# diffqc/dqc

Measured on AMD Instinct MI355X. Metric: SCF iterations/sec (Fock build + XC grid) per GPU, cc-pVDZ 20-atom, higher is better.
Workload: dtype f64

## Files before the change

dqc_amd/csrc/jk.hip:

```cpp
#include <cstdlib>

#include "common.hpp"

namespace dqc {

DQC_DEV void decode_tri(long long t, int &a, int &b) {
    long long r = (long long)((sqrt(8.0 * (double)t + 1.0) - 1.0) * 0.5);
    while (r * (r + 1) / 2 > t) r--;
    while ((r + 1) * (r + 2) / 2 <= t) r++;
    a = (int)r;
    b = (int)(t - r * (r + 1) / 2);
}

DQC_DEV void tile_load_patch(const double *__restrict__ tiles, int IJ, int KL, int I, int J, int K, int L, int r0, int c0, double2 &a0, double2 &b0, double2 &a1, double2 &b1, double2 &a2,
                             double2 &b2, double2 &a3, double2 &b3, const TileLay &ly) {
    const bool dr = I == J, dc = K == L;
    const double *tp = tiles + tile_base(I, J, K, KL, ly);
    const bool trunc = I == ly.last && ly.wl < 8;
    if (!dr && !dc) {
        if (trunc && r0 >= 8 * ly.wl) {
            a0 = b0 = a1 = b1 = a2 = b2 = a3 = b3 = make_double2(0.0, 0.0);
            return;
        }
        const double *q = tp + r0 * 64 + c0;
// ... 116 lines not shown
    if ((long long)blockIdx.x < ntiles) JKM_LOAD(blockIdx.x)
    for (long long T = blockIdx.x; T < ntiles; T += gridDim.x) {
        int IJ, KL, I, J, K, L;
        decode_tri(T, IJ, KL);
        decode_tri(IJ, I, J);
        decode_tri(KL, K, L);
        const double f = (I == J ? 0.5 : 1.0) * (K == L ? 0.5 : 1.0) * (IJ == KL ? 0.5 : 1.0);
        const int kk = c0 >> 3, l0 = c0 & 7, ii = r0 >> 3, j0 = r0 & 7;
        double g[4][4];
        g[0][0] = na0.x; g[0][1] = na0.y; g[0][2] = nb0.x; g[0][3] = nb0.y;
        g[1][0] = na1.x; g[1][1] = na1.y; g[1][2] = nb1.x; g[1][3] = nb1.y;
        g[2][0] = na2.x; g[2][1] = na2.y; g[2][2] = nb2.x; g[2][3] = nb2.y;
        g[3][0] = na3.x; g[3][1] = na3.y; g[3][2] = nb3.x; g[3][3] = nb3.y;
        if (T + gridDim.x < ntiles) JKM_LOAD(T + gridDim.x)
        if (NK) {
#pragma unroll
            for (int r = 0; r < 4; r++) {
                *reinterpret_cast<double2 *>(&s_g[(r0 + r) * LDT + c0]) = make_double2(g[r][0], g[r][1]);
                *reinterpret_cast<double2 *>(&s_g[(r0 + r) * LDT + c0 + 2]) = make_double2(g[r][2], g[r][3]);
            }
            const int blk = t >> 6, e = t & 63, x = e >> 3, y = e & 7;
            const int R = (blk & 1) ? I : J, Cb = (blk & 2) ? L : K;
#pragma unroll
            for (int q = 0; q < NK; q++) s_d[blk][x * 9 + y][q] = Dk[q * n2 + (size_t)(R * 8 + x) * npad + Cb * 8 + y];
        }
        for (int q = 0; q < nj; q++) {
            const double *dklp = Dj + q * n2 + (size_t)(K * 8 + kk) * npad + L * 8 + l0;
            const double *dijp = Dj + q * n2 + (size_t)(I * 8 + ii) * npad + J * 8 + j0;
            double dkl[4], dij[4];
#pragma unroll
            for (int c = 0; c < 4; c++) { dkl[c] = dklp[c]; dij[c] = dijp[c]; }
            double rs[4] = {0, 0, 0, 0}, cs[4] = {0, 0, 0, 0};
#pragma unroll
            for (int r = 0; r < 4; r++)
#pragma unroll
                for (int c = 0; c < 4; c++) {
                    rs[r] += g[r][c] * dkl[c];
                    cs[c] += g[r][c] * dij[r];
                }
#pragma unroll
            for (int r = 0; r < 4; r++) {
                double v = rs[r];
                v += __shfl_xor(v, 1); v += __shfl_xor(v, 2); v += __shfl_xor(v, 4); v += __shfl_xor(v, 8);
                rs[r] = v;
            }
#pragma unroll
            for (int c = 0; c < 4; c++) {
                double v = cs[c];
                v += __shfl_xor(v, 16); v += __shfl_xor(v, 32);
                cs[c] = v;
            }
            double *Jq = Jacc + q * n2;
            if ((lane & 15) == 0) {
#pragma unroll
                for (int r = 0; r < 4; r++) acc_add(&Jq[(size_t)(I * 8 + ii) * npad + J * 8 + j0 + r], 2.0 * f * rs[r], dsc);
            }
            if (lane < 16) {
#pragma unroll
                for (int c = 0; c < 4; c++) s_col[q & 1][wave][c0 + c] = cs[c];
            }
            __syncthreads();
            if (t < 64) {
                const double v = s_col[q & 1][0][t] + s_col[q & 1][1][t] + s_col[q & 1][2][t] + s_col[q & 1][3][t];
                acc_add(&Jq[(size_t)(K * 8 + (t >> 3)) * npad + L * 8 + (t & 7)], 2.0 * f * v, dsc);
            }
        }
        if (NK) {
            if (nj == 0) __syncthreads();
            const int o = t >> 2, pg = t & 3, x = o >> 3, y = o & 7, yh = y >> 2;
            double k1[NKD], k2[NKD], k3[NKD], k4[NKD];
#pragma unroll
            for (int q = 0; q < NK; q++) k1[q] = k2[q] = k3[q] = k4[q] = 0.0;
#pragma unroll 1
            for (int u = 0; u < 2; u++) {
                const int qq = pg + 4 * u, q4 = pg + 4 * (u ^ yh);
#pragma unroll 4
                for (int a = 0; a < 8; a++) {
                    const double g1 = s_g[(x * 8 + a) * LDT + qq * 8 + y], g2 = s_g[(a * 8 + x) * LDT + qq * 8 + y];
                    const double g3 = s_g[(x * 8 + a) * LDT + y * 8 + q4], g4 = s_g[(a * 8 + x) * LDT + y * 8 + q4];
                    if constexpr (NK == 2) {
                        const vd2 d1 = *reinterpret_cast<const vd2 *>(&s_d[0][a * 9 + qq][0]);
                        const vd2 d2 = *reinterpret_cast<const vd2 *>(&s_d[1][a * 9 + qq][0]);
                        const vd2 d3 = *reinterpret_cast<const vd2 *>(&s_d[2][a * 9 + q4][0]);
                        const vd2 d4 = *reinterpret_cast<const vd2 *>(&s_d[3][a * 9 + q4][0]);
                        k1[0] += g1 * d1.x; k1[1] += g1 * d1.y;
                        k2[0] += g2 * d2.x; k2[1] += g2 * d2.y;
                        k3[0] += g3 * d3.x; k3[1] += g3 * d3.y;
                        k4[0] += g4 * d4.x; k4[1] += g4 * d4.y;
                    } else {
#pragma unroll
                        for (int q = 0; q < NK; q++) {
                            k1[q] += g1 * s_d[0][a * 9 + qq][q];
                            k2[q] += g2 * s_d[1][a * 9 + qq][q];
                            k3[q] += g3 * s_d[2][a * 9 + q4][q];
                            k4[q] += g4 * s_d[3][a * 9 + q4][q];
                        }
                    }
                }
            }
#pragma unroll
            for (int q = 0; q < NK; q++) {
                double a1 = k1[q], a2 = k2[q], a3 = k3[q], a4 = k4[q];
                a1 += __shfl_xor(a1, 1); a1 += __shfl_xor(a1, 2);
                a2 += __shfl_xor(a2, 1); a2 += __shfl_xor(a2, 2);
                a3 += __shfl_xor(a3, 1); a3 += __shfl_xor(a3, 2);
                a4 += __shfl_xor(a4, 1); a4 += __shfl_xor(a4, 2);
                if (pg == 0) {
                    double *Kq = Kacc + q * n2;
                    acc_add(&Kq[(size_t)(I * 8 + x) * npad + L * 8 + y], f * a1, dsc);
                    acc_add(&Kq[(size_t)(J * 8 + x) * npad + L * 8 + y], f * a2, dsc);
                    acc_add(&Kq[(size_t)(I * 8 + x) * npad + K * 8 + y], f * a3, dsc);
                    acc_add(&Kq[(size_t)(J * 8 + x) * npad + K * 8 + y], f * a4, dsc);
                }
            }
        }
        __syncthreads();
    }
}

#undef JKM_LOAD
__global__ void jk_multi_prep_kernel(double *__restrict__ work, const double *__restrict__ dmj, int nj, const double *__restrict__ dmk,
                                     int nk, int nao, int npad, unsigned kanti) {
    const size_t n2 = (size_t)npad * npad, nn = (size_t)nao * nao;
    const int nd = nj + nk;
    for (size_t e = (size_t)blockIdx.x * blockDim.x + threadIdx.x; e < n2 * nd; e += (size_t)gridDim.x * blockDim.x) {
        const int q = e / n2;
        const size_t r = e - (size_t)q * n2;
        const int i = r / npad, j = r % npad;
        const double *dm = q < nj ? dmj + (size_t)q * nn : dmk + (size_t)(q - nj) * nn;
        double v = 0.0;
        const bool anti = q >= nj && ((kanti >> (q - nj)) & 1u);
        if (i < nao && j < nao) v = anti ? 0.5 * (dm[(size_t)i * nao + j] - dm[(size_t)j * nao + i]) : 0.5 * (dm[(size_t)i * nao + j] + dm[(size_t)j * nao + i]);
        work[e] = v;
        work[n2 * nd + e] = 0.0;
    }
}

__global__ void jk_multi_finish_kernel(double *__restrict__ J, int nj, double *__restrict__ K, int nk, const double *__restrict__ work,
                                       int nao, int npad, const double *__restrict__ dscp, unsigned kanti) {
    const double dsc = dscp ? *dscp : 0.0;
    const size_t n2 = (size_t)npad * npad, nn = (size_t)nao * nao;
    const double *acc = work + (size_t)(nj + nk) * n2;
    for (size_t e = (size_t)blockIdx.x * blockDim.x + threadIdx.x; e < nn * (nj + nk); e += (size_t)gridDim.x * blockDim.x) {
        const int q = e / nn;
        const size_t r = e - (size_t)q * nn;
        const int i = r / nao, j = r % nao;
        const double a = det_value(acc[q * n2 + (size_t)i * npad + j], dsc), at = det_value(acc[q * n2 + (size_t)j * npad + i], dsc);
        const double v = (q >= nj && ((kanti >> (q - nj)) & 1u)) ? a - at : a + at;
        if (q < nj) J[e] = v;
        else K[e - (size_t)nj * nn] = v;
    }
}

__global__ __launch_bounds__(256, 1) void j_stream_kernel(const double *__restrict__ dscp, const double *__restrict__ tiles,
                                                         double *__restrict__ work, int npad, long long ntiles, long long per_block,
                                                         long long tbeg, int nao) {
    const TileLay ly(nao);
    const double dsc = dscp ? *dscp : 0.0;
    __shared__ double s_col[2][4][64];
    const size_t n2 = (size_t)npad * npad;
    const double *Dp = work;
    double *Jacc = work + n2;
    const int t = threadIdx.x, lane = t & 63, wave = t >> 6;
    const int r0 = 4 * (t >> 4), c0 = 4 * (t & 15);
    const int kk = c0 >> 3, l0 = c0 & 7, ii = r0 >> 3, j0 = r0 & 7;
    const long long T0 = tbeg + (long long)blockIdx.x * per_block, T1 = min(T0 + per_block, ntiles);
    if (T0 >= T1) return;
    int IJ, KL, I, J, K, L;
    decode_tri(T0, IJ, KL);
    decode_tri(IJ, I, J);
    double rsacc[4] = {0, 0, 0, 0}, dij[4];
    {
        const double *dijp = Dp + (size_t)(I * 8 + ii) * npad + J * 8 + j0;
#pragma unroll
        for (int q = 0; q < 4; q++) dij[q] = dijp[q];
    }
    auto flush_rows = [&]() {
        const double fI = (I == J ? 0.5 : 1.0);
#pragma unroll
        for (int r = 0; r < 4; r++) {
            double v = rsacc[r];
            v += __shfl_xor(v, 1); v += __shfl_xor(v, 2); v += __shfl_xor(v, 4); v += __shfl_xor(v, 8);
            if ((lane & 15) == 0) acc_add(&Jacc[(size_t)(I * 8 + ii) * npad + J * 8 + j0 + r], 2.0 * fI * v, dsc);
            rsacc[r] = 0.0;
        }
    };
    int par = 0;
    for (long long T = T0; T < T1; T++, KL++) {
        if (KL > IJ) {
            flush_rows();
            IJ++;
            KL = 0;
            decode_tri(IJ, I, J);
            const double *dijp = Dp + (size_t)(I * 8 + ii) * npad + J * 8 + j0;
#pragma unroll
            for (int q = 0; q < 4; q++) dij[q] = dijp[q];
        }
        decode_tri(KL, K, L);
        const double fk = (K == L ? 0.5 : 1.0) * (IJ == KL ? 0.5 : 1.0);
        const double *dklp = Dp + (size_t)(K * 8 + kk) * npad + L * 8 + l0;
        double dkl[4];
#pragma unroll
        for (int q = 0; q < 4; q++) dkl[q] = fk * dklp[q];
        double cs[4] = {0, 0, 0, 0};
        {
            double2 ta0, tb0, ta1, tb1, ta2, tb2, ta3, tb3;
            tile_load_patch(tiles, IJ, KL, I, J, K, L, r0, c0, ta0, tb0, ta1, tb1, ta2, tb2, ta3, tb3, ly);
#define DQC_JS_ROW(R_, A_, B_)                                                                           \
    rsacc[R_] += A_.x * dkl[0] + A_.y * dkl[1] + B_.x * dkl[2] + B_.y * dkl[3];                          \
    cs[0] += A_.x * dij[R_]; cs[1] += A_.y * dij[R_]; cs[2] += B_.x * dij[R_]; cs[3] += B_.y * dij[R_];
            DQC_JS_ROW(0, ta0, tb0) DQC_JS_ROW(1, ta1, tb1) DQC_JS_ROW(2, ta2, tb2) DQC_JS_ROW(3, ta3, tb3)
#undef DQC_JS_ROW
        }
#pragma unroll
        for (int c = 0; c < 4; c++) {
            double v = cs[c];
            v += __shfl_xor(v, 16); v += __shfl_xor(v, 32);
            cs[c] = v;
        }
        if (lane < 16) {
#pragma unroll
            for (int c = 0; c < 4; c++) s_col[par][wave][c0 + c] = cs[c];
        }
        __syncthreads();
        if (t < 64) {
            const double v = s_col[par][0][t] + s_col[par][1][t] + s_col[par][2][t] + s_col[par][3][t];
            acc_add(&Jacc[(size_t)(K * 8 + (t >> 3)) * npad + L * 8 + (t & 7)], 2.0 * (I == J ? 0.5 : 1.0) * fk * v, dsc);
        }
        par ^= 1;
    }
    flush_rows();
}


__global__ __launch_bounds__(256, 4) void jk_stream_kernel(const double *__restrict__ dscp, const double *__restrict__ tiles,
                                                          double *__restrict__ work, int npad, long long ntiles, long long per_block,
                                                          long long tbeg, int nao) {
    const TileLay ly(nao);
    const double dsc = dscp ? *dscp : 0.0;
    constexpr int LDT = 68;
    __shared__ double s_col[4][64];
    __shared__ __attribute__((aligned(16))) double s_g[64 * LDT];
    __shared__ __attribute__((aligned(16))) double s_d[2][72][2];
    const size_t n2 = (size_t)npad * npad;
    const double *Dp = work;
    double *Jacc = work + n2, *Kacc = work + 2 * n2;
    const int t = threadIdx.x, lane = t & 63, wave = t >> 6;
    const int r0 = 4 * (t >> 4), c0 = 4 * (t & 15);
    const int kk = c0 >> 3, l0 = c0 & 7, ii = r0 >> 3, j0 = r0 & 7;
    const int o = t >> 2, pg = t & 3, x = o >> 3, y = o & 7, yh = y >> 2;
    const long long T0 = tbeg + (long long)blockIdx.x * per_block, T1 = min(T0 + per_block, ntiles);
    if (T0 >= T1) return;
    int IJ, KL, I, J, K, L;
    decode_tri(T0, IJ, KL);
    decode_tri(IJ, I, J);
    decode_tri(KL, K, L);
    double rsacc[4] = {0, 0, 0, 0}, dij[4];
    double k3acc = 0.0, k4acc = 0.0;
    {
        const double *dijp = Dp + (size_t)(I * 8 + ii) * npad + J * 8 + j0;
#pragma unroll
        for (int q = 0; q < 4; q++) dij[q] = dijp[q];
    }
    auto flush_rows = [&]() {
        const double fI = (I == J ? 0.5 : 1.0);
#pragma unroll
        for (int r = 0; r < 4; r++) {
            double v = rsacc[r];
            v += __shfl_xor(v, 1); v += __shfl_xor(v, 2); v += __shfl_xor(v, 4); v += __shfl_xor(v, 8);
            if ((lane & 15) == 0) acc_add(&Jacc[(size_t)(I * 8 + ii) * npad + J * 8 + j0 + r], 2.0 * fI * v, dsc);
            rsacc[r] = 0.0;
        }
    };
    auto flush_k34 = [&]() {
        double a3 = k3acc, a4 = k4acc;
        a3 += __shfl_xor(a3, 1); a3 += __shfl_xor(a3, 2);
        a4 += __shfl_xor(a4, 1); a4 += __shfl_xor(a4, 2);
        if (pg == 0) {
            acc_add(&Kacc[(size_t)(I * 8 + x) * npad + K * 8 + y], a3, dsc);
            acc_add(&Kacc[(size_t)(J * 8 + x) * npad + K * 8 + y], a4, dsc);
        }
        k3acc = k4acc = 0.0;
    };
    for (long long T = T0; T < T1; T++) {
        const double f = (I == J ? 0.5 : 1.0) * (K == L ? 0.5 : 1.0) * (IJ == KL ? 0.5 : 1.0);
        const double fk = (K == L ? 0.5 : 1.0) * (IJ == KL ? 0.5 : 1.0);
        const double *dklp = Dp + (size_t)(K * 8 + kk) * npad + L * 8 + l0;
        double dkl[4];
#pragma unroll
        for (int q = 0; q < 4; q++) dkl[q] = fk * dklp[q];
        double cs[4] = {0, 0, 0, 0};
        {
            double2 ta0, tb0, ta1, tb1, ta2, tb2, ta3, tb3;
            tile_load_patch(tiles, IJ, KL, I, J, K, L, r0, c0, ta0, tb0, ta1, tb1, ta2, tb2, ta3, tb3, ly);
#define DQC_JS_ROW(R_, A_, B_)                                                                           \
    rsacc[R_] += A_.x * dkl[0] + A_.y * dkl[1] + B_.x * dkl[2] + B_.y * dkl[3];                          \
    cs[0] += A_.x * dij[R_]; cs[1] += A_.y * dij[R_]; cs[2] += B_.x * dij[R_]; cs[3] += B_.y * dij[R_]; \
    *reinterpret_cast<double2 *>(&s_g[(r0 + R_) * LDT + c0]) = A_;                                       \
    *reinterpret_cast<double2 *>(&s_g[(r0 + R_) * LDT + c0 + 2]) = B_;
            DQC_JS_ROW(0, ta0, tb0) DQC_JS_ROW(1, ta1, tb1) DQC_JS_ROW(2, ta2, tb2) DQC_JS_ROW(3, ta3, tb3)
#undef DQC_JS_ROW
        }
        {
            const int blk = t >> 6, e = t & 63, xx = e >> 3, yy = e & 7;
            const int R = (blk & 1) ? I : J, Cb = (blk & 2) ? L : K;
            s_d[blk >> 1][xx * 9 + yy][blk & 1] = Dp[(size_t)(R * 8 + xx) * npad + Cb * 8 + yy];
        }
#pragma unroll
        for (int c = 0; c < 4; c++) {
            double v = cs[c];
            v += __shfl_xor(v, 16); v += __shfl_xor(v, 32);
            cs[c] = v;
        }
        if (lane < 16) {
#pragma unroll
            for (int c = 0; c < 4; c++) s_col[wave][c0 + c] = cs[c];
        }
        __syncthreads();
        if (t < 64) {
            const double v = s_col[0][t] + s_col[1][t] + s_col[2][t] + s_col[3][t];
            acc_add(&Jacc[(size_t)(K * 8 + (t >> 3)) * npad + L * 8 + (t & 7)], 2.0 * (I == J ? 0.5 : 1.0) * fk * v, dsc);
        }
        {
            double k1 = 0, k2 = 0, k3 = 0, k4 = 0;
#pragma unroll 1
            for (int u = 0; u < 2; u++) {
                const int q = pg + 4 * u, q4 = pg + 4 * (u ^ yh);
#pragma unroll
                for (int a = 0; a < 8; a++) {
                    typedef double vd2_ __attribute__((ext_vector_type(2)));
                    const vd2_ d12 = *reinterpret_cast<const vd2_ *>(&s_d[0][a * 9 + q][0]);
                    const vd2_ d34 = *reinterpret_cast<const vd2_ *>(&s_d[1][a * 9 + q4][0]);
                    k1 += s_g[(x * 8 + a) * LDT + q * 8 + y] * d12.x;
                    k2 += s_g[(a * 8 + x) * LDT + q * 8 + y] * d12.y;
                    k3 += s_g[(x * 8 + a) * LDT + y * 8 + q4] * d34.x;
                    k4 += s_g[(a * 8 + x) * LDT + y * 8 + q4] * d34.y;
                }
            }
            k1 += __shfl_xor(k1, 1); k1 += __shfl_xor(k1, 2);
            k2 += __shfl_xor(k2, 1); k2 += __shfl_xor(k2, 2);
            if (pg == 0) {
                acc_add(&Kacc[(size_t)(I * 8 + x) * npad + L * 8 + y], f * k1, dsc);
                acc_add(&Kacc[(size_t)(J * 8 + x) * npad + L * 8 + y], f * k2, dsc);
            }
            k3acc += f * k3;
            k4acc += f * k4;
        }
        if (T + 1 < T1) {
            if (KL == IJ) {
                flush_rows();
                flush_k34();
                IJ++;
                KL = 0; K = 0; L = 0;
                decode_tri(IJ, I, J);
                const double *dijp = Dp + (size_t)(I * 8 + ii) * npad + J * 8 + j0;
#pragma unroll
                for (int q = 0; q < 4; q++) dij[q] = dijp[q];
            } else {
                KL++;
                if (L == K) { flush_k34(); K++; L = 0; }
                else L++;
            }
        }
        __syncthreads();
    }
    flush_rows();
    flush_k34();
}

template <int NJ, int NK>
__global__ __launch_bounds__(256, 3) void jk_multi_stream_kernel(const double *__restrict__ dscp, const double *__restrict__ tiles,
                                                                double *__restrict__ work, int npad, long long ntiles,
                                                                long long per_block, int nao) {
    const TileLay ly(nao);
    const double dsc = dscp ? *dscp : 0.0;
    constexpr int LDT = 68;
    __shared__ double s_col[4][64];
    __shared__ __attribute__((aligned(16))) double s_g[64 * LDT];
    __shared__ __attribute__((aligned(16))) double s_d[4][72][NK];
    const size_t n2 = (size_t)npad * npad;
    const double *Dp = work, *Dk = work + (size_t)NJ * n2;
    double *Jacc = work + (size_t)(NJ + NK) * n2, *Kacc = Jacc + (size_t)NJ * n2;
// ... 37 lines not shown
                acc_add(&Kacc[q * n2 + (size_t)(I * 8 + x) * npad + K * 8 + y], a3, dsc);
                acc_add(&Kacc[q * n2 + (size_t)(J * 8 + x) * npad + K * 8 + y], a4, dsc);
            }
            k3acc[q] = k4acc[q] = 0.0;
        }
    };
    for (long long T = T0; T < T1; T++) {
        const double f = (I == J ? 0.5 : 1.0) * (K == L ? 0.5 : 1.0) * (IJ == KL ? 0.5 : 1.0);
        const double fk = (K == L ? 0.5 : 1.0) * (IJ == KL ? 0.5 : 1.0);
        const double *dklp = Dp + (size_t)(K * 8 + kk) * npad + L * 8 + l0;
        double dkl[4];
#pragma unroll
        for (int q = 0; q < 4; q++) dkl[q] = NJ ? fk * dklp[q] : 0.0;
        double cs[4] = {0, 0, 0, 0};
        {
            double2 ta0, tb0, ta1, tb1, ta2, tb2, ta3, tb3;
            tile_load_patch(tiles, IJ, KL, I, J, K, L, r0, c0, ta0, tb0, ta1, tb1, ta2, tb2, ta3, tb3, ly);
#define DQC_JS_ROW(R_, A_, B_)                                                                           \
    if (NJ) {                                                                                            \
        rsacc[R_] += A_.x * dkl[0] + A_.y * dkl[1] + B_.x * dkl[2] + B_.y * dkl[3];                      \
        cs[0] += A_.x * dij[R_]; cs[1] += A_.y * dij[R_]; cs[2] += B_.x * dij[R_]; cs[3] += B_.y * dij[R_]; \
    }                                                                                                    \
    *reinterpret_cast<double2 *>(&s_g[(r0 + R_) * LDT + c0]) = A_;                                       \
    *reinterpret_cast<double2 *>(&s_g[(r0 + R_) * LDT + c0 + 2]) = B_;
            DQC_JS_ROW(0, ta0, tb0) DQC_JS_ROW(1, ta1, tb1) DQC_JS_ROW(2, ta2, tb2) DQC_JS_ROW(3, ta3, tb3)
#undef DQC_JS_ROW
        }
        {
            const int blk = t >> 6, e = t & 63, xx = e >> 3, yy = e & 7;
            const int R = (blk & 1) ? I : J, Cb = (blk & 2) ? L : K;
#pragma unroll
            for (int q = 0; q < NK; q++) s_d[blk][xx * 9 + yy][q] = Dk[q * n2 + (size_t)(R * 8 + xx) * npad + Cb * 8 + yy];
        }
        if (NJ) {
#pragma unroll
            for (int c = 0; c < 4; c++) {
                double v = cs[c];
                v += __shfl_xor(v, 16); v += __shfl_xor(v, 32);
                cs[c] = v;
            }
            if (lane < 16) {
#pragma unroll
                for (int c = 0; c < 4; c++) s_col[wave][c0 + c] = cs[c];
            }
        }
        __syncthreads();
        if (NJ && t < 64) {
            const double v = s_col[0][t] + s_col[1][t] + s_col[2][t] + s_col[3][t];
            acc_add(&Jacc[(size_t)(K * 8 + (t >> 3)) * npad + L * 8 + (t & 7)], 2.0 * (I == J ? 0.5 : 1.0) * fk * v, dsc);
        }
        {
            double k1[NK], k2[NK], k3[NK], k4[NK];
#pragma unroll
            for (int q = 0; q < NK; q++) k1[q] = k2[q] = k3[q] = k4[q] = 0.0;
#pragma unroll 1
            for (int u = 0; u < 2; u++) {
                const int qq = pg + 4 * u, q4 = pg + 4 * (u ^ yh);
#pragma unroll 4
                for (int a = 0; a < 8; a++) {
                    const double g1 = s_g[(x * 8 + a) * LDT + qq * 8 + y], g2 = s_g[(a * 8 + x) * LDT + qq * 8 + y];
                    const double g3 = s_g[(x * 8 + a) * LDT + y * 8 + q4], g4 = s_g[(a * 8 + x) * LDT + y * 8 + q4];
#pragma unroll
                    for (int q = 0; q < NK; q++) {
                        k1[q] += g1 * s_d[0][a * 9 + qq][q];
                        k2[q] += g2 * s_d[1][a * 9 + qq][q];
                        k3[q] += g3 * s_d[2][a * 9 + q4][q];
                        k4[q] += g4 * s_d[3][a * 9 + q4][q];
                    }
                }
            }
#pragma unroll
            for (int q = 0; q < NK; q++) {
                double a1 = k1[q], a2 = k2[q];
                a1 += __shfl_xor(a1, 1); a1 += __shfl_xor(a1, 2);
                a2 += __shfl_xor(a2, 1); a2 += __shfl_xor(a2, 2);
                if (pg == 0) {
                    acc_add(&Kacc[q * n2 + (size_t)(I * 8 + x) * npad + L * 8 + y], f * a1, dsc);
                    acc_add(&Kacc[q * n2 + (size_t)(J * 8 + x) * npad + L * 8 + y], f * a2, dsc);
                }
                k3acc[q] += f * k3[q];
                k4acc[q] += f * k4[q];
            }
        }
        if (T + 1 < T1) {
            if (KL == IJ) {
                flush_rows();
                flush_k34();
                IJ++;
                KL = 0; K = 0; L = 0;
                decode_tri(IJ, I, J);
                if (NJ) {
                    const double *dijp = Dp + (size_t)(I * 8 + ii) * npad + J * 8 + j0;
#pragma unroll
                    for (int q = 0; q < 4; q++) dij[q] = dijp[q];
                }
            } else {
                KL++;
                if (L == K) { flush_k34(); K++; L = 0; }
                else L++;
            }
        }
        __syncthreads();
    }
    flush_rows();
    flush_k34();
}


}

extern "C" {

size_t dqc_jk_work_doubles(int nao) {
    const size_t npad = (size_t)(nao + DQC_TILE_B - 1) / DQC_TILE_B * DQC_TILE_B;
    return 5 * npad * npad + 8 + 128;
}

long long dqc_eri_tile_offset(int nao, long long tile) {
    using namespace dqc;
    const long long nt = (long long)dqc_eri_tile_count(nao);
    if (nao <= 0 || tile <= 0) return 0;
    if (tile >= nt) return eri_store_data_doubles(nao);
    auto tri = [](long long t, long long &a, long long &b) {
        long long r = (long long)((std::sqrt(8.0 * (double)t + 1.0) - 1.0) * 0.5);
        while (r * (r + 1) / 2 > t) r--;
        while ((r + 1) * (r + 2) / 2 <= t) r++;
        a = r;
        b = t - r * (r + 1) / 2;
    };
    long long IJ, KL, I, J, K, L;
    tri(tile, IJ, KL);
    tri(IJ, I, J);
    tri(KL, K, L);
    return tile_base((int)I, (int)J, (int)K, (int)KL, TileLay(nao));
}

int dqc_jk_from_tiles(double *d_J, double *d_K, const double *d_tiles, const double *d_dm, int nao,
                      double *d_work, void *stream) {
    return dqc_jk_from_tiles_part(d_J, d_K, d_tiles, d_dm, nao, d_work, 0, (long long)dqc_eri_tile_count(nao), stream);
}

static int jk_from_tiles_impl(double *d_J, double *d_K, const double *d_tiles_part, const double *d_dm, int nao, double *d_work,
                              long long tile_begin, long long tile_end, int with_k_prepared, void *stream);

int dqc_jk_from_tiles_part(double *d_J, double *d_K, const double *d_tiles_part, const double *d_dm, int nao, double *d_work,
                           long long tile_begin, long long tile_end, void *stream) {
    return jk_from_tiles_impl(d_J, d_K, d_tiles_part, d_dm, nao, d_work, tile_begin, tile_end, 0, stream);
}

int dqc_jk_stream_prepared(const double *d_tiles, int nao, double *d_work, int with_k, void *stream) {
    return jk_from_tiles_impl(nullptr, nullptr, d_tiles, nullptr, nao, d_work, 0, (long long)dqc_eri_tile_count(nao), with_k ? 1 : 0, stream);
}

static int jk_from_tiles_impl(double *d_J, double *d_K, const double *d_tiles_part, const double *d_dm, int nao, double *d_work,
                              long long tile_begin, long long tile_end, int with_k_prepared, void *stream) {
    using namespace dqc;
    if (nao <= 0) return DQC_OK;
    hipStream_t st = (hipStream_t)stream;
    const int npad = (nao + DQC_TILE_B - 1) / DQC_TILE_B * DQC_TILE_B;
    const long long nt_all = (long long)dqc_eri_tile_count(nao);
    if (tile_begin < 0 || tile_end > nt_all || tile_begin > tile_end) { set_error("dqc_jk_from_tiles_part: tile range outside the store"); return DQC_EINVAL; }
    const bool whole = tile_begin == 0 && tile_end == nt_all;
    if (!whole && deterministic_mode()) {
        set_error("dqc_jk_from_tiles_part: the deterministic mode needs the whole store (its scale reads the diagonal tiles)");
        return DQC_EINVAL;
    }
    const double *d_tiles = d_tiles_part - dqc_eri_tile_offset(nao, tile_begin);
    const long long ntiles = tile_end, tbeg = tile_begin, nrun = tile_end - tile_begin;
    const int with_k = d_dm ? (d_K != nullptr) : with_k_prepared;
    if (d_dm) {
        hipLaunchKernelGGL(jk_prep_kernel, dim3(64), dim3(256), 0, st, d_work, d_dm, nao, npad, with_k);
        DQC_CHECK_LAUNCH();
    }
    double *dscp = nullptr;
    if (deterministic_mode()) {
        dscp = d_work + 3 * (size_t)npad * npad;
        hipLaunchKernelGGL(jk_det_scale_kernel, dim3(1), dim3(256), 0, st, dscp, d_work, 1, (size_t)npad * npad, d_tiles, nao);
        DQC_CHECK_LAUNCH();
    }
    if (nrun == 0) {
    } else if (with_k) {
        static const long long jk_nblk_env = [] { const char *e = getenv("DQC_JK_NBLK"); return e ? atoll(e) : 0LL; }();
        const long long nblk = jk_nblk_env > 0 ? std::min<long long>(nrun, jk_nblk_env) : std::min<long long>(nrun, std::max<long long>(1024, std::min<long long>(6144, nrun / 8)));
        const long long per = (nrun + nblk - 1) / nblk;
        hipLaunchKernelGGL(jk_stream_kernel, dim3((unsigned)((nrun + per - 1) / per)), dim3(256), 0, st, dscp, d_tiles, d_work, npad, ntiles, per, tbeg, nao);
    } else {
        static const long long j_nblk_env = [] { const char *e = getenv("DQC_J_NBLK"); return e ? atoll(e) : 0LL; }();
        const long long nblk = std::max<long long>(1, std::min<long long>((nrun + 3) / 4, j_nblk_env > 0 ? j_nblk_env : 65536));
        const long long per = (nrun + nblk - 1) / nblk;
        hipLaunchKernelGGL(j_stream_kernel, dim3((unsigned)((nrun + per - 1) / per)), dim3(256), 0, st, dscp, d_tiles, d_work, npad, ntiles, per, tbeg, nao);
    }
    DQC_CHECK_LAUNCH();
    if (d_J) {
        hipLaunchKernelGGL(jk_finish_kernel, dim3(64), dim3(256), 0, st, d_J, d_K, d_work, nao, npad, dscp);
        DQC_CHECK_LAUNCH();
    }
    return DQC_OK;
}

size_t dqc_jk_multi_work_doubles(int nao, int nj, int nk) {
    const size_t npad = (size_t)(nao + DQC_TILE_B - 1) / DQC_TILE_B * DQC_TILE_B;
    return 2 * (size_t)(nj + (nk > 2 ? 2 : nk)) * npad * npad + 8;
}

static int jk_from_tiles_multi_impl(double *d_J, const double *d_dmJ, int nj, double *d_K, const double *d_dmK, int nk, const int *k_antisym,
                                    const double *d_tiles, int nao, double *d_work, void *stream);

int dqc_jk_from_tiles_multi(double *d_J, const double *d_dmJ, int nj, double *d_K, const double *d_dmK, int nk,
                            const double *d_tiles, int nao, double *d_work, void *stream) {
    return jk_from_tiles_multi_impl(d_J, d_dmJ, nj, d_K, d_dmK, nk, nullptr, d_tiles, nao, d_work, stream);
}

int dqc_jk_from_tiles_multi_asym(double *d_J, const double *d_dmJ, int nj, double *d_K, const double *d_dmK, int nk, const int *k_antisym,
                                 const double *d_tiles, int nao, double *d_work, void *stream) {
    return jk_from_tiles_multi_impl(d_J, d_dmJ, nj, d_K, d_dmK, nk, k_antisym, d_tiles, nao, d_work, stream);
}

static int jk_from_tiles_multi_impl(double *d_J, const double *d_dmJ, int nj, double *d_K, const double *d_dmK, int nk, const int *k_antisym,
                                    const double *d_tiles, int nao, double *d_work, void *stream) {
    using namespace dqc;
    if (nao <= 0 || (nj <= 0 && nk <= 0)) return DQC_OK;
    if (nj < 0 || nk < 0) { set_error("dqc_jk_from_tiles_multi: negative matrix count"); return DQC_EINVAL; }
    hipStream_t st = (hipStream_t)stream;
    const int npad = (nao + DQC_TILE_B - 1) / DQC_TILE_B * DQC_TILE_B;
    const size_t nn = (size_t)nao * nao;
    const long long ntiles = (long long)dqc_eri_tile_count(nao);
    const unsigned grid = (unsigned)std::min<long long>(ntiles, 256 * 16);
    int kdone = 0, first = 1;
    while (first || kdone < nk) {
        const int njp = first ? nj : 0, nkp = std::min(2, nk - kdone);
        unsigned kanti = 0;
        for (int q = 0; k_antisym && q < nkp; q++) kanti |= k_antisym[kdone + q] ? 1u << q : 0u;
        hipLaunchKernelGGL(jk_multi_prep_kernel, dim3(64), dim3(256), 0, st, d_work, d_dmJ, njp, d_dmK + (size_t)kdone * nn, nkp, nao, npad, kanti);
        DQC_CHECK_LAUNCH();
        double *dscp = nullptr;
        if (deterministic_mode()) {
            dscp = d_work + 2 * (size_t)(njp + nkp) * npad * npad;
            hipLaunchKernelGGL(jk_det_scale_kernel, dim3(1), dim3(256), 0, st, dscp, d_work, njp + nkp, (size_t)npad * npad, d_tiles, nao);
            DQC_CHECK_LAUNCH();
        }
        const long long nblk_s = std::min<long long>(ntiles, std::max<long long>(1024, std::min<long long>(6144, ntiles / 8)));
        const long long per_s = (ntiles + nblk_s - 1) / nblk_s;
        const dim3 grid_s((unsigned)((ntiles + per_s - 1) / per_s));
        const bool stream_ok = njp <= 1 && nkp >= 1;
        if (stream_ok && njp == 1 && nkp == 2) hipLaunchKernelGGL((jk_multi_stream_kernel<1, 2>), grid_s, dim3(256), 0, st, dscp, d_tiles, d_work, npad, ntiles, per_s, nao);
        else if (stream_ok && njp == 1 && nkp == 1) hipLaunchKernelGGL((jk_multi_stream_kernel<1, 1>), grid_s, dim3(256), 0, st, dscp, d_tiles, d_work, npad, ntiles, per_s, nao);
        else if (stream_ok && njp == 0 && nkp == 2) hipLaunchKernelGGL((jk_multi_stream_kernel<0, 2>), grid_s, dim3(256), 0, st, dscp, d_tiles, d_work, npad, ntiles, per_s, nao);
        else if (stream_ok && njp == 0 && nkp == 1) hipLaunchKernelGGL((jk_multi_stream_kernel<0, 1>), grid_s, dim3(256), 0, st, dscp, d_tiles, d_work, npad, ntiles, per_s, nao);
        else if (nkp == 2) hipLaunchKernelGGL(jk_multi_kernel<2>, dim3(grid), dim3(256), 0, st, dscp, d_tiles, d_work, npad, ntiles, njp, nao);
        else if (nkp == 1) hipLaunchKernelGGL(jk_multi_kernel<1>, dim3(grid), dim3(256), 0, st, dscp, d_tiles, d_work, npad, ntiles, njp, nao);
        else hipLaunchKernelGGL(jk_multi_kernel<0>, dim3(grid), dim3(256), 0, st, dscp, d_tiles, d_work, npad, ntiles, njp, nao);
        DQC_CHECK_LAUNCH();
        hipLaunchKernelGGL(jk_multi_finish_kernel, dim3(64), dim3(256), 0, st, d_J, njp, d_K + (size_t)kdone * nn, nkp, d_work, nao, npad, dscp, kanti);
        DQC_CHECK_LAUNCH();
        kdone += nkp;
        first = 0;
    }
    return DQC_OK;
}

}
```

dqc_amd/hamilton.py:

```python
from collections import namedtuple
from typing import List, Optional

import os

import torch

from . import lib
from .basis import make_tables
from .linop import LinearOperator
from .utils.datastruct import AtomCGTOBasis, SpinParam, ValGrad
from .xc import LibXC, exx_fraction_of

_COULOMB_SIDE = {}


def register_coulomb_side_stream(grid_stream, side_stream):
    key = (grid_stream.device.index, grid_stream.cuda_stream)
    if side_stream is None:
        _COULOMB_SIDE.pop(key, None)
    else:
        _COULOMB_SIDE[key] = side_stream


class _Memo:

    def __init__(self, size=1):
        self.size, self.rows = size, []

    def get(self, *keys):
        for ks, vs, val in self.rows:
            if all(a is b for a, b in zip(ks, keys)) and vs == tuple(k._version for k in keys):
                return val
        return None

    def put(self, val, *keys):
        self.rows = [(keys, tuple(k._version for k in keys), val)] + self.rows[:self.size - 1]
        return val

    def drop(self, val):
        self.rows = [r for r in self.rows if r[2] is not val]

    def clear(self):
        self.rows = []


class _Factor:
    __slots__ = ("orb", "w", "pairs")

    def __init__(self, orb, w, pairs=None):
        self.orb, self.w, self.pairs = orb, w, pairs


_Energies = namedtuple("_Energies", "j xc k ka", defaults=(None, None, None, None))


try:
    from dqc.hamilton.base_hamilton import BaseHamilton as _Base
except Exception:
    _Base = object


_SIDE_STREAMS = {}


def _side_stream(dev):
    key = torch.device(dev).index if torch.device(dev).index is not None else torch.cuda.current_device()
    if key not in _SIDE_STREAMS:
        _SIDE_STREAMS[key] = torch.cuda.Stream(device=dev)
    return _SIDE_STREAMS[key]


class HamiltonMI355(_Base):
    def __init__(self, atombases: List[AtomCGTOBasis], spherical: bool = True, df=None, efield=None,
                 vext: Optional[torch.Tensor] = None, cache=None, orthozer: bool = True,
                 aoparamzer: str = "qr", device="cuda"):
        if not spherical:
            raise NotImplementedError("only spherical AOs (the reference default) are implemented on MI355X")
        self._dfoptions = df
        if efield is not None:
            if isinstance(efield, torch.Tensor):
                efield = (efield,)
            if len(efield) > 2:
                raise NotImplementedError("electric-field terms beyond the field gradient (int1e r0r0r0...) are not implemented")
            for i, ef in enumerate(efield):
                assert ef.numel() == 3 ** (i + 1), "The %d-th tuple element of efield must have %d elements" % (i, 3 ** (i + 1))
        self._efield = efield
        if aoparamzer not in ("qr", "matexp"):
            raise RuntimeError("Unknown ao parameterizer: %s. Available options are: ['qr', 'matexp']" % aoparamzer)
        lib.load()
        self.device = torch.device(device)
        if self.device.type != "cuda":
            raise lib.DqcAmdError("HamiltonMI355 needs a ROCm device ('cuda'); there is no CPU path")
        self.dtype = torch.float64
        self.atombases = atombases
        self.spherical = spherical
        atm, bas, env, zs = make_tables(atombases)
        self._tab = lib.Tables(atm, bas, env)
        self._zs = zs
        self._nao_ao = self._tab.nao
        self._ld = lib.padded_nao(self._nao_ao)
        self._lda = lib.ao_stride(self._nao_ao)

        self._ovlp_ao = lib.int1e("ovlp", self._tab, self.device)
        self._X = None
        self._fill_done = None
        self._eri_mode = os.environ.get("DQC_AMD_ERI", "auto")
        if self._eri_mode not in ("auto", "tiles", "direct"):
            raise RuntimeError("DQC_AMD_ERI must be auto, tiles or direct")
        self._direct = False
        self.orthogonalized = bool(orthozer)
        if df is None:
            self._df = None
        else:
            from .df import DFMI355
            self._df = DFMI355(df, atombases, self._orthozer, self.device)
        self._vext = vext
        self.is_grid_set = False
        self.is_ao_set = False
        self.is_grad_ao_set = False
        self.is_built = False
        self.xc = None
        self.xcfamily = 1
        self._fuse_k = False
        self._jk_memo, self._jkpol_memo, self._energy_memo, self._factors = _Memo(), _Memo(), _Memo(), _Memo(2)
        self._dfk_memo = _Memo(2)
        self._w_checked = _Memo(2)
        self.grid_path_counts = {"factor": 0, "dense": 0}

    def clear_memos(self):
        for m in (self._jk_memo, self._jkpol_memo, self._energy_memo, self._factors, self._dfk_memo):
            m.clear()

    @property
    def _orthozer(self):
        if self._X is None:
            if self.orthogonalized:
                ev, evec = torch.linalg.eigh(self._ovlp_ao)
                acc = ev > 1e-6
                self._X = evec[:, acc] * ev[acc] ** (-0.5)
            else:
                self._X = torch.eye(self._nao_ao, dtype=self.dtype, device=self.device)
        return self._X

    @property
    def _tiles(self):
        ev = self._fill_done
        if ev is not None and not torch.cuda.is_current_stream_capturing():
            if ev.query():
                self._fill_done = None
            else:
                torch.cuda.current_stream(self.device).wait_event(ev)
        t = self._tiles_store
        if t is not None and not torch.cuda.is_current_stream_capturing():
            cur = torch.cuda.current_stream(self.device)
            seen = self.__dict__.setdefault("_tile_streams", set())
            if cur.cuda_stream not in seen:
                seen.add(cur.cuda_stream)
                t.record_stream(cur)
        return t

    @property
    def nao(self) -> int:
        return self._orthozer.shape[-1]

    @property
    def kpts(self):
        raise TypeError("Isolated molecule Hamiltonian does not have kpts property")

    @property
    def df(self):
        return self._df

    def _convert2(self, mat):
        return self._orthozer.transpose(-2, -1) @ mat @ self._orthozer

    def _unconvert_dm(self, dm):
        return self._orthozer @ dm @ self._orthozer.transpose(-2, -1)

    def build(self):
        if self.is_built:
            return self
        tab, dev = self._tab, self.device
        fill_done = None
        if self._df is None:
            need = lib.eri_store_doubles(tab.nao) * 8
            if self._pworld > 1 and self._eri_mode == "tiles":
                self._tile_slice = lib.tile_slice(tab.nao, self._prank, self._pworld)
                need = self._tile_slice[2] * 8
            free, _total = torch.cuda.mem_get_info(dev)
            free += torch.cuda.memory_reserved(dev) - torch.cuda.memory_allocated(dev)
            mode = self._eri_mode
            if mode == "auto":
                mode = "tiles" if need <= free else "direct"
            if mode == "tiles" and need > free:
                raise lib.DqcAmdError(
                    "the exact-J/K ERI tile store of this basis needs %.1f GB (nao = %d) but only %.1f GB of device memory "
                    "are free: use eri='direct' (DQC_AMD_ERI=direct: the integrals are re-evaluated in every Fock build) or the "
                    "density-fitted Coulomb operator (mol.densityfit(method='coulomb', auxbasis=...))" % (need / 1e9, tab.nao, free / 1e9))
            self._direct = mode == "direct"
            if self._eri_mode == "auto" and self._direct:
                import warnings
                warnings.warn("the ERI tile store of this basis (nao = %d: %.1f GB) does not fit the %.1f GB of device memory that are "
                              "free: direct SCF (integrals re-evaluated in every Fock build, no hipGraph / lockstep step); "
                              "DQC_AMD_ERI=tiles insists on the store" % (tab.nao, need / 1e9, free / 1e9))
            self.eri_mode_used = mode
            if self._direct and self.xc is not None:
                self._check_hybrid(exx_fraction_of(self.xc))
        if self._df is None and self._direct:
            self._tiles_store, self._jkwork = None, None
            self._dctx = lib.DirectContext(tab, dev)
            self._dinc = {}
        elif self._df is None:
            main = torch.cuda.current_stream(dev)
            side = _side_stream(dev)
            side.wait_stream(main)
            with torch.cuda.stream(side):
                if self._tile_slice is not None:
                    self._tiles_store = lib.eri_tiles_part(tab, dev, self._tile_slice[0], self._tile_slice[1])
                else:
                    self._tiles_store = lib.eri_tiles(tab, dev)
                fill_done = torch.cuda.Event()
                fill_done.record(side)
            self._tiles_store.record_stream(main)
            self._fill_done = fill_done
            self._jkwork = lib.jk_workspace(self._nao_ao, dev)
        kin = lib.int1e("kin", tab, dev)
        nuc = lib.int1e("nuc", tab, dev, self._zs)
        self.olp_mat = self._convert2(self._ovlp_ao)
        if self._efield is not None:
            fac = 1.0
            for i, ef in enumerate(self._efield):
                fac *= i + 1
                mats = lib.int1e("r0" * (i + 1), tab, dev)
                kin = kin + torch.einsum("dab,d->ab", mats, ef.reshape(-1).to(device=dev, dtype=self.dtype)) / fac
        self.kinnucl_mat = self._convert2(kin + nuc)
        self.nucl_mat = self._convert2(nuc)
        if self._df is not None:
            self._df.build()
        self.is_built = True
        if self._vext is not None:
            self.kinnucl_mat = self.kinnucl_mat + self.get_vext(self._vext.to(self.device)).fullmatrix()
        return self

    def setup_grid(self, grid, xc=None) -> None:
        family = 1 if xc is None else xc.family
        if family not in (1, 2, 4):
            raise RuntimeError("unknown xc family %s" % family)
        self._check_hybrid(exx_fraction_of(xc))
        if self.is_grid_set and getattr(self, "grid", None) is grid and family == self.xcfamily:
            if xc is not self.xc:
                self._energy_memo.clear()
                self._jk_memo.clear()
            self.xc = xc
            return
        self.xc = xc
        self.xcfamily = family
        self.grid = grid
        assert grid.coord_type == "cart"
        self.rgrid = grid.get_rgrid().to(self.device)
        self.dvolume = grid.get_dvolume().to(self.device).contiguous()
        self.ngrid_full = int(self.rgrid.shape[0])
        self.live_index = None
        if os.environ.get("DQC_AMD_PRUNE_GRID", "1") != "0" and self.ngrid_full > 0:
            cached = getattr(grid, "_live_index_cache", None)
            if cached is None or cached[0].device != self.dvolume.device:
                idx = torch.nonzero(self.dvolume != 0).squeeze(1)
                cached = (idx, int(idx.shape[0]))
                try:
                    grid._live_index_cache = cached
                except AttributeError:
                    pass
            if cached[1] < self.ngrid_full:
                self.live_index = cached[0]
                self.rgrid = self.rgrid[self.live_index].contiguous()
                self.dvolume = self.dvolume[self.live_index].contiguous()
        if self._pworld > 1:
            g = self.rgrid.shape[0]
            lo, hi = g * self._prank // self._pworld, g * (self._prank + 1) // self._pworld
            self.rgrid, self.dvolume = self.rgrid[lo:hi].contiguous(), self.dvolume[lo:hi].contiguous()
        deriv = {1: 0, 2: 1, 4: 2}[self.xcfamily]
        self._ao = lib.eval_gto(self._tab, self.rgrid, deriv)
        self.is_grid_set = True
        self.is_ao_set = True
        self.is_grad_ao_set = deriv >= 1
        self.is_lapl_ao_set = deriv == 2
        self._ao_lapl_pm = None

    def _check_hybrid(self, a):
        if a == 0.0:
            return
        if self._df is not None and not self._df.exchange:
            raise NotImplementedError("hybrid functionals (exact-exchange fraction %g) cannot be used with density fitting: "
                                      "Mol.densityfit() fits the Coulomb operator J only, there is no fitted exchange "
                                      "(densityfit(exchange=True) fits K as well)" % a)
        if self._pworld > 1:
            raise NotImplementedError("hybrid functionals (exact-exchange fraction %g) on a Hamiltonian sharded over several GPUs "
                                      "(shard_over) are not implemented" % a)
        if self._eri_mode == "direct" or (self.is_built and self._direct):
            raise NotImplementedError("hybrid functionals (exact-exchange fraction %g) with direct SCF (DQC_AMD_ERI=direct) are not "
                                      "implemented: the incremental J / K builds are not wired to the hybrid Fock build" % a)

    @property
    def exx_fraction(self):
        return exx_fraction_of(self.xc)

    def grid_select(self, x):
        return x if self.live_index is None else x[..., self.live_index]

    def grid_scatter(self, x):
        if self.live_index is None:
            return x
        out = torch.zeros(tuple(x.shape[:-1]) + (self.ngrid_full,), dtype=x.dtype, device=x.device)
        out[..., self.live_index] = x
        return out

    @property
    def basis(self):
        a = self._ao if self._ao.dim() == 2 else self._ao[0]
        return a[:, :self._nao_ao]

    @property
    def grad_basis(self):
        return self._ao[1:4, :, :self._nao_ao]

    def get_nuclattr(self):
        return LinearOperator.m(self.nucl_mat, is_hermitian=True)

    def get_kinnucl(self):
        return LinearOperator.m(self.kinnucl_mat, is_hermitian=True)

    def get_overlap(self):
        return LinearOperator.m(self.olp_mat, is_hermitian=True)

    def _batched(self, fcn, dm):
        if dm.dim() == 2:
            return fcn(dm)
        bshape = dm.shape[:-2]
        res = [fcn(d) for d in dm.reshape(-1, *dm.shape[-2:])]
        return torch.stack(res).reshape(*bshape, *res[0].shape)

    def _jk_orth(self, dm, need_k):
        c = self._jk_memo.get(dm)
        if c is not None and (c[1] is not None or not need_k):
            return c
        dao = self._unconvert_dm(dm)
        with_k = need_k or self._fuse_k
        J, K = self._jk_ao(dao, with_k)
        return self._jk_memo.put((self._sym_orth(J), None if K is None else self._sym_orth(K)), dm)

    def use_direct_eri(self, on: bool = True):
        if self.is_built:
            raise RuntimeError("use_direct_eri must be called before build()")
        self._eri_mode = "direct" if on else "tiles"
        return self

    _pg, _prank, _pworld = None, 0, 1
    _tile_slice = None

    def shard_over(self, group=None, eri="direct"):
        import torch.distributed as dist
        if self.is_built or self.is_grid_set:
            raise RuntimeError("shard_over must be called before build() and setup_grid()")
        if self._df is not None or self._vext is not None:
            raise RuntimeError("a density-fitted Hamiltonian / one with an external potential on the grid cannot be sharded")
        if not (dist.is_available() and dist.is_initialized()):
            raise RuntimeError("shard_over needs an initialised torch.distributed process group")
        self._pg = group
        self._prank, self._pworld = dist.get_rank(group), dist.get_world_size(group)
        if eri not in ("direct", "tiles"):
            raise RuntimeError("shard_over: eri must be 'direct' or 'tiles'")
        if lib.load().dqc_get_deterministic():
            raise RuntimeError("shard_over: the deterministic mode (dqc_set_deterministic) covers unsharded Hamiltonians only")
        self._eri_mode = eri
        self._tile_slice = None
        return self

    @property
    def sharded(self):
        return self._pworld > 1

    @property
    def tiles_resident(self):
        return self._df is None and not self._direct and self._tile_slice is None

    _deferred = None
    _j_stream = None

    def _allsum(self, t):
        if self._pworld > 1 and t is not None:
            if self._deferred is not None:
                self._deferred.append(t)
                return t
            import torch.distributed as dist
            dist.all_reduce(t, op=dist.ReduceOp.SUM, group=self._pg)
        return t

    def _allsum_flush(self):
        ts, self._deferred = self._deferred, None
        if ts:
            import torch.distributed as dist
            flat = torch.cat([t.reshape(-1) for t in ts])
            dist.all_reduce(flat, op=dist.ReduceOp.SUM, group=self._pg)
            o = 0
            for t in ts:
                t.copy_(flat[o:o + t.numel()].reshape(t.shape))
                o += t.numel()

# ... 546 lines not shown
```

Before: 817.1.

## Stream J tiles with incremental pointers and nontemporal loads for large ERI sets

Rewrites the J-only streaming kernel so it walks the tile array with an incremental pointer and row/column counters. This replaces the per-tile triangular decode and the generic patch-loading helper. Columns are remapped to two contiguous pairs per thread so the shared-memory stores can use double2. A template variant issues nontemporal loads when the tile range exceeds 256 MiB, to avoid polluting cache with single-use data. Separately, the energy memo gets two slots and is cleared when the grid changes, which adds some risk of stale or inconsistent caching behaviour.

```diff
diff --git a/dqc_amd/csrc/jk.hip b/dqc_amd/csrc/jk.hip
--- a/dqc_amd/csrc/jk.hip
+++ b/dqc_amd/csrc/jk.hip
@@ -292,29 +292,50 @@
     }
 }
 
+template <bool ONCE>
+DQC_DEV double2 j_tile_load16(const double *p) {
+    if constexpr (ONCE) {
+        typedef double v2d_ __attribute__((ext_vector_type(2)));
+        const v2d_ v = __builtin_nontemporal_load(reinterpret_cast<const v2d_ *>(p));
+        return make_double2(v.x, v.y);
+    } else {
+        return *reinterpret_cast<const double2 *>(p);
+    }
+}
+
+template <bool ONCE>
 __global__ __launch_bounds__(256, 1) void j_stream_kernel(const double *__restrict__ dscp, const double *__restrict__ tiles,
                                                          double *__restrict__ work, int npad, long long ntiles, long long per_block,
                                                          long long tbeg, int nao) {
     const TileLay ly(nao);
     const double dsc = dscp ? *dscp : 0.0;
-    __shared__ double s_col[2][4][64];
+    __shared__ __attribute__((aligned(16))) double s_col[2][4][64];
     const size_t n2 = (size_t)npad * npad;
     const double *Dp = work;
     double *Jacc = work + n2;
     const int t = threadIdx.x, lane = t & 63, wave = t >> 6;
-    const int r0 = 4 * (t >> 4), c0 = 4 * (t & 15);
-    const int kk = c0 >> 3, l0 = c0 & 7, ii = r0 >> 3, j0 = r0 & 7;
+    const int r0 = 4 * (t >> 4), ii = r0 >> 3, j0 = r0 & 7;
+    const int cA = 2 * (t & 15), cB = 32 + cA;
     const long long T0 = tbeg + (long long)blockIdx.x * per_block, T1 = min(T0 + per_block, ntiles);
     if (T0 >= T1) return;
     int IJ, KL, I, J, K, L;
     decode_tri(T0, IJ, KL);
     decode_tri(IJ, I, J);
+    decode_tri(KL, K, L);
+    const double *tp = tiles + tile_base(I, J, K, KL, ly);
+    int R = 0;
+    unsigned prow[4];
     double rsacc[4] = {0, 0, 0, 0}, dij[4];
-    {
+    auto enter_pair = [&]() {
+        R = tile_rows(I, J, ly);
         const double *dijp = Dp + (size_t)(I * 8 + ii) * npad + J * 8 + j0;
 #pragma unroll
-        for (int q = 0; q < 4; q++) dij[q] = dijp[q];
-    }
+        for (int q = 0; q < 4; q++) {
+            dij[q] = dijp[q];
+            prow[q] = I == J ? tile_pidx(true, ii, j0 + q) : r0 + q;
+        }
+    };
+    enter_pair();
     auto flush_rows = [&]() {
         const double fI = (I == J ? 0.5 : 1.0);
 #pragma unroll
@@ -326,32 +347,41 @@
         }
     };
     int par = 0;
-    for (long long T = T0; T < T1; T++, KL++) {
-        if (KL > IJ) {
-            flush_rows();
-            IJ++;
-            KL = 0;
-            decode_tri(IJ, I, J);
-            const double *dijp = Dp + (size_t)(I * 8 + ii) * npad + J * 8 + j0;
-#pragma unroll
-            for (int q = 0; q < 4; q++) dij[q] = dijp[q];
-        }
-        decode_tri(KL, K, L);
-        const double fk = (K == L ? 0.5 : 1.0) * (IJ == KL ? 0.5 : 1.0);
-        const double *dklp = Dp + (size_t)(K * 8 + kk) * npad + L * 8 + l0;
-        double dkl[4];
-#pragma unroll
-        for (int q = 0; q < 4; q++) dkl[q] = fk * dklp[q];
+    for (long long T = T0;;) {
+        const bool dc = K == L;
+        const unsigned C = tile_dim(dc);
+        const double fk = (dc ? 0.5 : 1.0) * (IJ == KL ? 0.5 : 1.0);
+        const double *pa = Dp + (size_t)(K * 8 + (cA >> 3)) * npad + L * 8 + (cA & 7);
+        const double *pb = Dp + (size_t)(K * 8 + (cB >> 3)) * npad + L * 8 + (cB & 7);
+        const double dkl[4] = {fk * pa[0], fk * pa[1], fk * pb[0], fk * pb[1]};
+        const double2 z2 = make_double2(0.0, 0.0);
+        double2 ta0 = z2, tb0 = z2, ta1 = z2, tb1 = z2, ta2 = z2, tb2 = z2, ta3 = z2, tb3 = z2;
+        const bool ok0 = prow[0] < (unsigned)R, ok1 = prow[1] < (unsigned)R, ok2 = prow[2] < (unsigned)R, ok3 = prow[3] < (unsigned)R;
+        const double *q0 = tp + prow[0] * C, *q1 = tp + prow[1] * C, *q2 = tp + prow[2] * C, *q3 = tp + prow[3] * C;
+        if (!dc && R == tile_dim(I == J)) {
+            ta0 = j_tile_load16<ONCE>(q0 + cA); tb0 = j_tile_load16<ONCE>(q0 + cB);
+            ta1 = j_tile_load16<ONCE>(q1 + cA); tb1 = j_tile_load16<ONCE>(q1 + cB);
+            ta2 = j_tile_load16<ONCE>(q2 + cA); tb2 = j_tile_load16<ONCE>(q2 + cB);
+            ta3 = j_tile_load16<ONCE>(q3 + cA); tb3 = j_tile_load16<ONCE>(q3 + cB);
+        } else if (!dc) {
+            if (ok0) { ta0 = *reinterpret_cast<const double2 *>(q0 + cA); tb0 = *reinterpret_cast<const double2 *>(q0 + cB); }
+            if (ok1) { ta1 = *reinterpret_cast<const double2 *>(q1 + cA); tb1 = *reinterpret_cast<const double2 *>(q1 + cB); }
+            if (ok2) { ta2 = *reinterpret_cast<const double2 *>(q2 + cA); tb2 = *reinterpret_cast<const double2 *>(q2 + cB); }
+            if (ok3) { ta3 = *reinterpret_cast<const double2 *>(q3 + cA); tb3 = *reinterpret_cast<const double2 *>(q3 + cB); }
+        } else {
+            const int pc0 = tile_pidx(true, cA >> 3, cA & 7), pc1 = tile_pidx(true, cA >> 3, (cA & 7) + 1);
+            const int pc2 = tile_pidx(true, cB >> 3, cB & 7), pc3 = tile_pidx(true, cB >> 3, (cB & 7) + 1);
+            if (ok0) { ta0 = make_double2(q0[pc0], q0[pc1]); tb0 = make_double2(q0[pc2], q0[pc3]); }
+            if (ok1) { ta1 = make_double2(q1[pc0], q1[pc1]); tb1 = make_double2(q1[pc2], q1[pc3]); }
+            if (ok2) { ta2 = make_double2(q2[pc0], q2[pc1]); tb2 = make_double2(q2[pc2], q2[pc3]); }
+            if (ok3) { ta3 = make_double2(q3[pc0], q3[pc1]); tb3 = make_double2(q3[pc2], q3[pc3]); }
+        }
         double cs[4] = {0, 0, 0, 0};
-        {
-            double2 ta0, tb0, ta1, tb1, ta2, tb2, ta3, tb3;
-            tile_load_patch(tiles, IJ, KL, I, J, K, L, r0, c0, ta0, tb0, ta1, tb1, ta2, tb2, ta3, tb3, ly);
 #define DQC_JS_ROW(R_, A_, B_)                                                                           \
     rsacc[R_] += A_.x * dkl[0] + A_.y * dkl[1] + B_.x * dkl[2] + B_.y * dkl[3];                          \
     cs[0] += A_.x * dij[R_]; cs[1] += A_.y * dij[R_]; cs[2] += B_.x * dij[R_]; cs[3] += B_.y * dij[R_];
-            DQC_JS_ROW(0, ta0, tb0) DQC_JS_ROW(1, ta1, tb1) DQC_JS_ROW(2, ta2, tb2) DQC_JS_ROW(3, ta3, tb3)
+        DQC_JS_ROW(0, ta0, tb0) DQC_JS_ROW(1, ta1, tb1) DQC_JS_ROW(2, ta2, tb2) DQC_JS_ROW(3, ta3, tb3)
 #undef DQC_JS_ROW
-        }
 #pragma unroll
         for (int c = 0; c < 4; c++) {
             double v = cs[c];
@@ -359,15 +389,28 @@
             cs[c] = v;
         }
         if (lane < 16) {
-#pragma unroll
-            for (int c = 0; c < 4; c++) s_col[par][wave][c0 + c] = cs[c];
+            *reinterpret_cast<double2 *>(&s_col[par][wave][cA]) = make_double2(cs[0], cs[1]);
+            *reinterpret_cast<double2 *>(&s_col[par][wave][cB]) = make_double2(cs[2], cs[3]);
         }
         __syncthreads();
         if (t < 64) {
             const double v = s_col[par][0][t] + s_col[par][1][t] + s_col[par][2][t] + s_col[par][3][t];
             acc_add(&Jacc[(size_t)(K * 8 + (t >> 3)) * npad + L * 8 + (t & 7)], 2.0 * (I == J ? 0.5 : 1.0) * fk * v, dsc);
         }
+        if (++T >= T1) break;
         par ^= 1;
+        if (KL == IJ) {
+            flush_rows();
+            IJ++;
+            KL = 0; K = 0; L = 0;
+            if (++J > I) { I++; J = 0; }
+            tp = tiles + tile_base(I, J, 0, 0, ly);
+            enter_pair();
+        } else {
+            tp += (unsigned)R * C;
+            KL++;
+            if (++L > K) { K++; L = 0; }
+        }
     }
     flush_rows();
 }
@@ -711,6 +754,8 @@
     return jk_from_tiles_impl(nullptr, nullptr, d_tiles, nullptr, nao, d_work, 0, (long long)dqc_eri_tile_count(nao), with_k ? 1 : 0, stream);
 }
 
+constexpr long long J_ONCE_MIN_BYTES = 256LL << 20;
+
 static int jk_from_tiles_impl(double *d_J, double *d_K, const double *d_tiles_part, const double *d_dm, int nao, double *d_work,
                               long long tile_begin, long long tile_end, int with_k_prepared, void *stream) {
     using namespace dqc;
@@ -747,7 +792,8 @@
         static const long long j_nblk_env = [] { const char *e = getenv("DQC_J_NBLK"); return e ? atoll(e) : 0LL; }();
         const long long nblk = std::max<long long>(1, std::min<long long>((nrun + 3) / 4, j_nblk_env > 0 ? j_nblk_env : 65536));
         const long long per = (nrun + nblk - 1) / nblk;
-        hipLaunchKernelGGL(j_stream_kernel, dim3((unsigned)((nrun + per - 1) / per)), dim3(256), 0, st, dscp, d_tiles, d_work, npad, ntiles, per, tbeg, nao);
+        const bool once = 8 * (dqc_eri_tile_offset(nao, tile_end) - dqc_eri_tile_offset(nao, tile_begin)) > J_ONCE_MIN_BYTES;
+        hipLaunchKernelGGL(once ? j_stream_kernel<true> : j_stream_kernel<false>, dim3((unsigned)((nrun + per - 1) / per)), dim3(256), 0, st, dscp, d_tiles, d_work, npad, ntiles, per, tbeg, nao);
     }
     DQC_CHECK_LAUNCH();
     if (d_J) {
diff --git a/dqc_amd/hamilton.py b/dqc_amd/hamilton.py
--- a/dqc_amd/hamilton.py
+++ b/dqc_amd/hamilton.py
@@ -122,7 +122,7 @@
         self.xc = None
         self.xcfamily = 1
         self._fuse_k = False
-        self._jk_memo, self._jkpol_memo, self._energy_memo, self._factors = _Memo(), _Memo(), _Memo(), _Memo(2)
+        self._jk_memo, self._jkpol_memo, self._energy_memo, self._factors = _Memo(), _Memo(), _Memo(2), _Memo(2)
         self._dfk_memo = _Memo(2)
         self._w_checked = _Memo(2)
         self.grid_path_counts = {"factor": 0, "dense": 0}
@@ -253,6 +253,7 @@
                 self._jk_memo.clear()
             self.xc = xc
             return
+        self._energy_memo.clear()
         self.xc = xc
         self.xcfamily = family
         self.grid = grid
```

Result: faster. 833.1 (median of 6 runs) (+2.0%).
